# bhansconnect/alphazero-pybind11

Measured on AMD Instinct MI355X. Metric: self-play games/sec (whole node), Connect4 @ 800 MCTS sims, higher is better.
Workload: dtype bf16

## Files before the change

alphazero-pybind11_amd/csrc/dev_cache.h:

```cpp
#pragma once
#include <hip/hip_runtime.h>
#include <stdint.h>

#include <type_traits>

#include "dev_rng.h"

namespace azmi {

struct CacheView {
  uint32_t shards, cap, ghost_cap;
  uint32_t tcap, gcap;
  uint32_t np, nv;
  uint64_t* hashes;
  uint32_t* freq;
  float* policy;
  float* value;
  uint32_t* s_ring;
  uint32_t* m_ring;
  uint64_t* ghost_ring;
  uint32_t* state;
  uint64_t* map_key;
  uint32_t* map_val;
  uint64_t* gset_key;
// ... 280 lines not shown
    }
    g = uni(g);
    if (__ballot(have == cache_key(hash)) != 0ull) {
      if (g && lane == 0) __hip_atomic_store(locks + sh, 0u, __ATOMIC_RELAXED, __HIP_MEMORY_SCOPE_AGENT);
      return true;
    }
    if (g) { got = 1; break; }
    __builtin_amdgcn_s_sleep(8);
  }
  if (!got) return false;
  {
    WaveShardT<true> ws(c, sh, lane);
    const int slot = ws.insert(hash);
    if (slot >= 0) {
      const size_t e = static_cast<size_t>(sh) * kWaveCap + slot;
      if constexpr (PROBE_SAFE) {
        if (lane == 0) c_st<true>(c.hashes + e, 0ull);
        asm volatile("s_waitcnt vmcnt(0)" ::: "memory");
      }
      if (lane < c.np) c_st<true>(reinterpret_cast<uint32_t*>(c.policy) + e * c.np + lane, __float_as_uint(p_lane));
      if (lane < c.nv) c_st<true>(reinterpret_cast<uint32_t*>(c.value) + e * c.nv + lane, __float_as_uint(v_lane));
      if constexpr (PROBE_SAFE) asm volatile("s_waitcnt vmcnt(0)" ::: "memory");
      ws.store();
    }
  }
  asm volatile("s_waitcnt vmcnt(0)" ::: "memory");
  if (lane == 0) __hip_atomic_store(locks + sh, 0u, __ATOMIC_RELAXED, __HIP_MEMORY_SCOPE_AGENT);
  return true;
}

struct NoPreload { __device__ __forceinline__ void operator()() const {} };
template <int G, class F = NoPreload>
__device__ __forceinline__ int wave_shard_find(const CacheView& c, uint64_t hash, uint32_t glane, uint32_t* shard_out, F&& before_loads = F()) {
  const uint64_t k = cache_key(hash);
  const uint32_t sh = static_cast<uint32_t>(hash % c.shards);
  *shard_out = sh;
  const uint64_t* hs = c.hashes + static_cast<size_t>(sh) * kWaveCap;
  uint64_t hv[kWaveCap / G];
#pragma unroll
  for (int i = 0; i < static_cast<int>(kWaveCap) / G; ++i) hv[i] = hs[i * G + static_cast<int>(glane)];
  before_loads();
  int found = -1;
#pragma unroll
  for (int i = 0; i < static_cast<int>(kWaveCap) / G; ++i)
    if (hv[i] == k) found = i * G + static_cast<int>(glane);
  if constexpr (G == 8) {
    found = max(found, __builtin_amdgcn_update_dpp(0, found, 0xB1, 0xF, 0xF, true));
    found = max(found, __builtin_amdgcn_update_dpp(0, found, 0x4E, 0xF, 0xF, true));
    found = max(found, __builtin_amdgcn_update_dpp(0, found, 0x141, 0xF, 0xF, true));
  } else {
#pragma unroll
    for (int off = 1; off < G; off <<= 1) found = max(found, __shfl_xor(found, off, G));
  }
  return found;
}
__device__ inline void wave_shard_find_account(const CacheView& c, uint64_t hash, uint32_t sh, int slot) {
  unsigned long long* st = c.stats + static_cast<size_t>(sh) * 4;
  if (slot < 0) {
    atomicAdd(&st[1], 1ULL);
    if (c.ghost_cap > 0) {
      const uint64_t k = cache_key(hash);
      bool in_ghost = false;
      for (uint32_t i = 0; i < c.ghost_cap; ++i)
        in_ghost = in_ghost || (c.map_val[static_cast<size_t>(sh) * kWaveCap + i] &&
                                c.ghost_ring[static_cast<size_t>(sh) * c.ghost_cap + i] == k);
      if (in_ghost) atomicAdd(&st[3], 1ULL);
    }
    return;
  }
  atomicAdd(&st[0], 1ULL);
  uint32_t* f = c.freq + static_cast<size_t>(sh) * kWaveCap + slot;
  if (atomicAdd(f, 1u) >= 3u) atomicSub(f, 1u);
}


constexpr uint32_t kApplyMax = 8192;
template <uint32_t U = 8>
__device__ __forceinline__ void wave_copy_row(float* __restrict__ dst, const float* __restrict__ src, uint32_t n, uint32_t lane) {
  for (uint32_t e0 = 0; e0 < n; e0 += 64 * U) {
    float t[U];
#pragma unroll
    for (uint32_t u = 0; u < U; ++u) { const uint32_t e = e0 + u * 64 + lane; t[u] = e < n ? src[e] : 0.0f; }
#pragma unroll
    for (uint32_t u = 0; u < U; ++u) { const uint32_t e = e0 + u * 64 + lane; if (e < n) dst[e] = t[u]; }
  }
}
__device__ __forceinline__ void cache_apply_batch(const CacheView& c, const uint64_t* keys, const float* policy,
                                                   const float* value, uint32_t n, uint32_t* s_sid,
                                                   const uint8_t* groups = nullptr, uint32_t group = 0) {
  const uint32_t tid = threadIdx.x, wave = tid >> 6, lane = tid & 63;
  const uint32_t i = blockIdx.x * (blockDim.x >> 6) + wave;
  const bool own_rows = c.np <= 64 && c.nv <= 64;
  const uint64_t own_key = i < n ? keys[i] : 0ull;
  const float own_p = (i < n && own_rows && lane < c.np) ? policy[static_cast<size_t>(i) * c.np + lane] : 0.0f;
  const float own_v = (i < n && own_rows && lane < c.nv) ? value[static_cast<size_t>(i) * c.nv + lane] : 0.0f;
  for (uint32_t j = tid; j < n; j += blockDim.x) {
    const uint64_t k = (groups && groups[j] != group) ? 0 : keys[j];
    s_sid[j] = k ? static_cast<uint32_t>(k % c.shards) : 0xFFFFFFFFu;
  }
  __syncthreads();
  if (i >= n) return;
  const uint32_t my = s_sid[i];
  if (my == 0xFFFFFFFFu) return;
  bool earlier = false;
  for (uint32_t j = lane; j < i; j += 64) earlier = earlier || (s_sid[j] == my);
  if (__ballot(earlier)) return;
// ... 27 lines not shown
```

alphazero-pybind11_amd/csrc/engine_kernels.h:

```cpp
#pragma once
#include <hip/hip_runtime.h>
#include <stdint.h>

#include "dev_games.h"
#include "dev_rng.h"
#include "engine_types.h"

namespace azmi {

constexpr float kNoiseAlphaRatio = 10.83f;

__device__ __forceinline__ uint32_t seat_param(const uint32_t (&a)[4], uint32_t seat) {
  return seat == 0 ? a[0] : seat == 1 ? a[1] : seat == 2 ? a[2] : a[3];
}

__device__ __forceinline__ uint32_t gum_plan(uint32_t m, uint32_t n, uint32_t want, uint32_t& num_c_out, uint32_t& v_per_out) {
  num_c_out = 0; v_per_out = 0;
  if (m <= 1) { if (want == 0) { num_c_out = 1; v_per_out = n; } return 1; }
  uint32_t log2m = 0;
  for (uint32_t v = m - 1; v > 0; v >>= 1) ++log2m;
  if (log2m == 0) log2m = 1;
  const uint32_t d0 = n / (log2m * m);
  const uint32_t base_v = d0 > 1u ? d0 : 1u;
  uint32_t sims_used = 0, num_c = m, count = 0;
// ... 324 lines not shown
      const float sc = bcast(score_l, ci);
      if (sc > best_score) { best_score = sc; best = ci; }
    }
    return bcast(mv_l, best);
  }

  __device__ __forceinline__ bool expand_node(uint32_t seat, uint32_t node, const typename GM::State& st, uint64_t meta_keep,
                              uint32_t& c0_out, uint32_t& k_out, uint32_t* mv_out = nullptr) {
    const size_t tb = tree_base(seat);
    const uint32_t k = GM::num_valid(st);
    static_assert(GM::MAXK <= 8, "eight 4-bit move fields");
    uint32_t packed = 0;
    {
      uint32_t vm = GM::valid_mask(st), pos = 0;
      while (vm) { const uint32_t m = __builtin_ctz(vm); vm &= vm - 1; packed |= m << (4 * pos); ++pos; }
    }
    auto swap_fields = [&](uint32_t a, uint32_t b) {
      const uint32_t fa = (packed >> (4 * a)) & 0xFu, fb = (packed >> (4 * b)) & 0xFu;
      packed = (packed & ~((0xFu << (4 * a)) | (0xFu << (4 * b)))) | (fb << (4 * a)) | (fa << (4 * b));
    };
    if (k > 1) {
      uint32_t i = 1;
      if ((k & 1u) == 0) {
        const uint32_t j = lemire_below(rng, 2);
        swap_fields(i, j);
        ++i;
      }
      while (i != k) {
        const uint32_t swap_range = i + 1, b1 = swap_range + 1;
        const uint32_t x = lemire_below(rng, swap_range * b1);
        const uint32_t p0 = x / b1, p1 = x % b1;
        swap_fields(i, p0);
        ++i;
        swap_fields(i, p1);
        ++i;
      }
    }
    const uint32_t mv = lane < k ? (packed >> (4 * lane)) & 0xFu : 0u;
    const uint32_t c0 = AZMI_SEL(t_bump, seat);
    if (c0 + k > ep.cap) { raise(1u); return false; }
    if (lane < k) {
      const size_t ci = tb + c0 + lane;
      ar.nodes[ci].n = 0; ar.nodes[ci].q = 0.0f; ar.nodes[ci].pr = 0.0f; ar.nodes[ci].d = 0.0f; ar.nodes[ci].v = 0.0f;
      ar.nodes[ci].meta = meta_pack(0, 0, mv, 0, 0);
    }
#pragma unroll
    for (int p = 0; p < P; ++p) if (static_cast<uint32_t>(p) == seat) t_bump[p] = c0 + k;
    if (lane == 0)
      ar.nodes[tb + node].meta = meta_pack(c0, k, meta_mv(meta_keep), meta_player(meta_keep), meta_term(meta_keep));
    c0_out = c0;
    k_out = k;
    if (mv_out) *mv_out = mv;
    return true;
  }

  __device__ __forceinline__ uint32_t select_child(uint32_t k, uint32_t n_l, float q_l, float p_l, float v_parent,
                                   uint32_t n_parent, float fpu_reduction, uint32_t if_l = 0) const {
    return select_among(k, n_l, q_l, p_l, v_parent, select_parent(n_parent), ep.cpuct, fpu_reduction, if_l);
  }
  __device__ __forceinline__ static float select_parent(uint32_t n_parent) { return sqrtf(static_cast<float>(n_parent)); }
  __device__ __forceinline__ uint32_t select_among(uint32_t k, uint32_t n_l, float q_l, float p_l, float v_parent,
                                   float sqrt_n, float cpuct, float fpu_reduction, uint32_t if_l = 0) const {
    const float seen = seqsum8((lane < k && n_l > 0) ? p_l : 0.0f);
    const float fpu_value = v_parent - fpu_reduction * sqrtf(seen);
    float u = (n_l == 0 ? fpu_value : q_l) + cpuct * p_l * sqrt_n / static_cast<float>(n_l + if_l + 1);
    u = (u != u) ? ((lane == 0) ? __builtin_inff() : -__builtin_inff()) : u;
    u = (lane >= k) ? -__builtin_inff() : u;
    uint32_t idx = lane < k ? lane : 0xFFFFu;
    {
      float ou = dpp_f<0xB1>(u); uint32_t oi = dpp_u<0xB1>(idx);
      bool take = (ou > u) | ((ou == u) & (oi < idx));
      u = take ? ou : u; idx = take ? oi : idx;
      ou = dpp_f<0x4E>(u); oi = dpp_u<0x4E>(idx);
      take = (ou > u) | ((ou == u) & (oi < idx));
      u = take ? ou : u; idx = take ? oi : idx;
      ou = dpp_f<0x141>(u); oi = dpp_u<0x141>(idx);
      take = (ou > u) | ((ou == u) & (oi < idx));
      u = take ? ou : u; idx = take ? oi : idx;
    }
    return idx;
  }

  __device__ __forceinline__ bool find_leaf_wu(uint32_t seat, typename GM::State& leaf, uint32_t& term, uint32_t* nif) {
    sync_lanes();
    const size_t tb = tree_base(seat);
    const uint32_t root = AZMI_SEL(t_root, seat);
    cur = root; plen = 0;
    leaf = gs;
    uint64_t meta = ar.nodes[tb + cur].meta;
    uint32_t n = ar.nodes[tb + cur].n, nf = nif[cur];
    uint32_t* path = ar.path + static_cast<size_t>(slot) * ep.max_depth;
    while ((n > 0 || nf > 0) && meta_nch(meta) != 0 && meta_term(meta) == 0) {
      if (plen >= ep.max_depth) { raise(8u); return false; }
      if (lane == 0) path[plen] = cur;
      ++plen;
      const uint32_t k = meta_nch(meta), c0 = meta_ch0(meta);
      const size_t ci = tb + c0 + lane;
      uint32_t n_l = 0, if_l = 0; float q_l = 0.0f, p_l = 0.0f; uint64_t m_l = 0;
      if (lane < k) { n_l = ar.nodes[ci].n; q_l = ar.nodes[ci].q; p_l = ar.nodes[ci].pr; m_l = ar.nodes[ci].meta; if_l = nif[c0 + lane]; }
      const float fpu = (cur == root && seat_fpu_zero(seat)) ? 0.0f : ep.fpu_reduction;
      const uint32_t best = select_child(k, n_l, q_l, p_l, ar.nodes[tb + cur].v, n + nf, fpu, if_l);
      if (lane == 0) nif[cur] = nf + 1;
      cur = c0 + best;
      n = bcast(n_l, best);
      nf = bcast(if_l, best);
      meta = bcast(m_l, best);
// ... 618 lines not shown
#pragma unroll
      for (int j = 0; j < 3; ++j) { atomicAdd(reinterpret_cast<unsigned long long*>(&ar.a_cnt[j * S + slot]), static_cast<unsigned long long>(gc[j])); ar.g_cnt[j * S + slot] = 0; }
      atomicAdd(&ar.slot_games[slot], 1u);
      const uint32_t pos = atomicAdd(&ar.ctl->ended_count, 1u);
      ar.ended_list[pos] = slot;
    }
  }

  __device__ __forceinline__ void emit_leaf(const typename GM::State& leaf, uint64_t key) const {
    float* row = ar.canon + static_cast<size_t>(slot) * GM::CANON;
    for (uint32_t e = lane; e < static_cast<uint32_t>(GM::CANON); e += G) row[e] = GM::canonical_at(leaf, e);
    if (lane == 0) {
      ar.leaf_key[slot] = key;
      if (ar.leaf_pos) {
        ar.leaf_pos[0 * static_cast<size_t>(ep.S) + slot] = leaf.bb[0];
        ar.leaf_pos[1 * static_cast<size_t>(ep.S) + slot] = leaf.bb[1];
        ar.leaf_pos[2 * static_cast<size_t>(ep.S) + slot] = leaf.player;
      }
    }
  }
  struct NoEarly { __device__ __forceinline__ bool operator()(int, float&, float&) const { return false; } };
  struct NoAfter { __device__ __forceinline__ void operator()(float, float) const {} };
  template <class F = NoPreload, class E = NoEarly, class A = NoAfter>
  __device__ __forceinline__ bool cache_lookup(uint64_t key, uint32_t group, float& hit_pi, float& hit_v, F&& before_loads = F(), E&& early = E(),
                                               A&& after_hit = A()) const {
    uint32_t sh;
    const CacheView cache = ep.num_groups == 1 ? ar.cache : ar.caches[group];
    const int cslot = wave_shard_find<G>(cache, key, lane, &sh, before_loads);
    if (lane == 0) {
      unsigned long long* st = cache.stats + static_cast<size_t>(sh) * 4;
      if (cslot < 0) {
        atomicAdd(&st[1], 1ULL);
      } else {
        atomicAdd(&st[0], 1ULL);
        uint32_t* f = cache.freq + static_cast<size_t>(sh) * kWaveCap + cslot;
        atomicAdd(f, 1u);
        atomicMin(f, 3u);
      }
    }
    static_assert(M <= G, "one lane per policy entry");
    bool have = early(cslot, hit_pi, hit_v);
    if (!have) {
      if (cslot < 0) return false;
      const float* sp = cache.policy + (static_cast<size_t>(sh) * cache.cap + cslot) * M;
      const float* sv = cache.value + (static_cast<size_t>(sh) * cache.cap + cslot) * (P + 1);
      hit_pi = lane < static_cast<uint32_t>(M) ? sp[lane] : 0.0f;
      hit_v = lane <= static_cast<uint32_t>(P) ? sv[lane] : 0.0f;
      after_hit(hit_pi, hit_v);
    }
    if (lane < static_cast<uint32_t>(M)) ar.pi[static_cast<size_t>(slot) * M + lane] = hit_pi;
    if (lane <= static_cast<uint32_t>(P)) ar.v[static_cast<size_t>(slot) * (P + 1) + lane] = hit_v;
    return true;
  }
};

template <class GM, bool kPlayout = false, bool kMover = false>
__device__ __forceinline__ uint32_t round_slot(const EngineParams& ep, const EngineArrays& ar, const uint32_t slot, const uint32_t lane) {
  constexpr int G = GM::GROUP;
  constexpr int P = GM::P;
  if (slot >= ep.S) return 0xFFu;
  if (ar.ctl->stop) return 0xFFu;
  const uint8_t st = ar.sstate[slot];
  if (st == kSlotDone || st == kSlotEnded) { if (ep.cache_on && lane == 0) ar.cache_keys[slot] = 0; return 0xFFu; }
  if constexpr (!kMover) {
    if (st == kSlotQueued) {
      if (lane == 0) {
        const uint32_t group = ar.leaf_group[slot];
        if (ep.cache_on) ar.cache_keys[slot] = cache_key(ar.leaf_key[slot]);
        ar.eval_list[static_cast<size_t>(group) * ep.S + atomicAdd(&ar.ctl->eval_count[group], 1u)] = slot;
        ar.sstate[slot] = kSlotWaitEval;
      }
      return kSlotWaitEval;
    }
  }
  SlotCtx<GM> c(ep, ar, slot, lane);
  c.trace(100);
  c.load();
  if constexpr (kMover) c.flags &= ~kFlagListed;
  c.trace(101);
  uint32_t inline_sims = 0, insert_key_set = 0;
  PathRegs prec;
  bool need_process = (st == kSlotWaitEval);
  if (!need_process) {
    c.start_game();
    c.draw_capped();
    c.set_gumbel_target();
    if (ep.gumbel_on && st == kSlotRestart && !ep.tree_reuse) c.set_gumbel_num_sims(c.gs.player, 0);
  }
  bool have_regs = false;
  float reg_pi = 0.0f, reg_v = 0.0f;
  for (;;) {
    if (need_process) {
      const uint32_t cp = c.gs.player;
      const bool noise = c.seat_eps(cp) > 0 && !(c.flags & kFlagCapped);
      c.process_result(cp, (c.flags & kFlagLeafNeedsNet) != 0, noise, have_regs, reg_pi, reg_v);
      have_regs = false;
      c.trace(102);
      const uint32_t goal = (c.flags & kFlagCapped) ? c.seat_cap_visits(cp) : c.seat_visits(cp);
      if (AZMI_SEL(c.t_depth, cp) >= goal) {
        if (c.make_move(cp)) { if (ep.cache_on && lane == 0) ar.cache_keys[slot] = 0; c.store(kSlotEnded); c.trace(107); return kSlotEnded; }
        c.trace(103);
      }
    }
    const uint32_t cp = c.gs.player;
    typename GM::State leaf;
    uint32_t term = 0;
// ... 308 lines not shown
```

alphazero-pybind11_amd/csrc/pipe_types.h:

```cpp
#pragma once
#include <stdint.h>

namespace azmi {

constexpr uint32_t kReqGranules = 4;
constexpr uint32_t kResStride = 16;
constexpr uint32_t kResV = 7;
constexpr uint32_t kPipeRing = 32768;
enum PipeErr : uint32_t { kPipeErrTimeout = 1, kPipeErrRing = 2, kPipeErrTag = 4, kPipeErrLog = 8, kPipeErrLock = 16, kPipeErrSlots = 32, kPipeErrNetTimeout = 64 };

__host__ __device__ inline uint64_t pipe_lap_tag(uint32_t pos) { return static_cast<uint64_t>(((pos / kPipeRing) & 0x7FFFu) + 1u); }
__host__ __device__ inline uint64_t pipe_mix64(uint64_t x) { x ^= x >> 30; x *= 0xBF58476D1CE4E5B9ULL; x ^= x >> 27; x *= 0x94D049BB133111EBULL; x ^= x >> 31; return x; }
constexpr unsigned long long kPipeGroupSalt = 0xA5A5A5A55A5A5A5AULL;
__host__ __device__ inline uint32_t pipe_l0_entry(uint64_t key, uint32_t mask) { return static_cast<uint32_t>(pipe_mix64(key ^ 0x5851F42D4C957F2DULL)) & mask; }
__host__ __device__ inline uint32_t pipe_l0_tag(uint64_t key, uint32_t k) { return static_cast<uint32_t>(pipe_mix64(key + 0x9E3779B97F4A7C15ULL * (k + 1u)) >> 32) | 1u; }
__host__ __device__ inline uint64_t pipe_lap_tag_r(uint32_t pos, uint32_t shift) { return static_cast<uint64_t>(((pos >> shift) & 0x7FFFu) + 1u); }
constexpr unsigned long long kTokMove = 0x8000ull;
constexpr unsigned long long kTokSlotMask = 0x7FFFull;

struct PipeWg {
  uint32_t rhead;
  uint32_t rtail;
  uint32_t pad[30];
};
static_assert(sizeof(PipeWg) == 128, "one line");

struct PipeCtl {
  uint32_t head; uint32_t pad0[31];
  uint32_t tail; uint32_t pad1[31];
  uint32_t head1; uint32_t pad4[31];
  uint32_t tail1; uint32_t pad5[31];
  uint32_t err;
  uint32_t pad6[31];
  unsigned long long freezes, freeze_max;
  unsigned long long tile_hist[6];
  uint32_t pad7[16];
  uint32_t pad2a, pad2;
  unsigned long long tiles;
  unsigned long long tile_boards;
  unsigned long long epochs;
  unsigned long long sims_total;
  unsigned long long l0_hits;
  uint32_t lost_total, pad3;
  uint32_t dbg[18];
  unsigned long long prof[16];
};
static_assert(sizeof(PipeCtl) == 1024, "eight lines");

struct PipeEpoch {
  unsigned long long sims; uint32_t pad0[30];
  unsigned long long t0;
  uint32_t stop;
  uint32_t tree_done;
  uint32_t tree_arrived, net_arrived;
  uint32_t tree_late, net_late;
  uint32_t tree_late_n, net_late_n;
  uint32_t reserved[2];
  uint32_t pad1[20];
  uint32_t ins_count;
  uint32_t ended;
  uint32_t dead;
  uint32_t ins_done;
  uint32_t moved;
  uint32_t lost;
  uint32_t pad2[26];
};
static_assert(sizeof(PipeEpoch) == 384, "memset block: three lines");

struct PipeArrays {
  PipeCtl* ctl;
  PipeEpoch* ep;
  unsigned long long* ring;
  unsigned long long* ring1;
  uint32_t n_groups;
  uint32_t net_groups;
  uint32_t lock_base1;
  uint8_t* ins_grp;
  unsigned long long* rring;
  PipeWg* wg;
  uint32_t rshift;
  uint32_t big_at;
  uint32_t census_hold;
  uint32_t take_wait;
  uint32_t max_inline;
  uint32_t min_active;
  unsigned long long* res;
  unsigned long long* l0;
  uint32_t l0_mask;
  uint32_t test_drop;
// ... 16 lines not shown
```

alphazero-pybind11_amd/csrc/pipeline.hip:

```cpp
#include <hip/hip_runtime.h>

#include <chrono>
#include <mutex>
#include <cstdio>
#include <cstdlib>
#include <cstring>
#include <map>
#include <memory>

#include "../../include/azmi.h"
#include "engine_host.h"
#include "engine_kernels.h"
#include "leafnet_c4.h"
#include "pipe_types.h"

using namespace azmi;

namespace azmi {

__device__ __forceinline__ unsigned long long g_ld(const unsigned long long* p) { return __hip_atomic_load(p, __ATOMIC_RELAXED, __HIP_MEMORY_SCOPE_AGENT); }
__device__ __forceinline__ uint32_t g_ld(const uint32_t* p) { return __hip_atomic_load(p, __ATOMIC_RELAXED, __HIP_MEMORY_SCOPE_AGENT); }
__device__ __forceinline__ void g_st(unsigned long long* p, unsigned long long v) { __hip_atomic_store(p, v, __ATOMIC_RELAXED, __HIP_MEMORY_SCOPE_AGENT); }
__device__ __forceinline__ void g_st(uint32_t* p, uint32_t v) { __hip_atomic_store(p, v, __ATOMIC_RELAXED, __HIP_MEMORY_SCOPE_AGENT); }

// ... 94 lines not shown
  {
    const unsigned long long em = __ballot(on && lane == 0 && res_state == kSlotEnded);
    const unsigned long long dm = __ballot(on && lane == 0 && (res_state == kSlotDone || res_state == 0xFFu));
    const unsigned long long om = __ballot(on && lane == 0);
    const unsigned long long sm = __ballot(on && lane == 0 && was_sim != 0u);
    if (wlane == 0) {
      if (em) atomicAdd(&pe->ended, static_cast<uint32_t>(__popcll(em)));
      if (dm) atomicAdd(&pe->dead, static_cast<uint32_t>(__popcll(dm)));
      if (sm) atomicAdd(&pe->sims, static_cast<unsigned long long>(__popcll(sm)));
      atomicAdd(&pe->moved, static_cast<uint32_t>(__popcll(om)));
    }
  }
  return res_state;
}

#ifndef AZMI_TREE_MINB
#define AZMI_TREE_MINB 2
#endif
template <class GM, int NT, bool PROF, bool TWO = false, bool GUM = false>
__global__ __launch_bounds__(NT, AZMI_TREE_MINB) void k_pipe_tree(PipeKernArgs ka) {
  constexpr int G = GM::GROUP;
  constexpr int P = GM::P;
  static_assert(P == 2 && G == 8 && GM::M == 7, "written for Connect4's 8-lane groups");
  const EngineParams& ep = ka.ep;
  const EngineArrays& ar = ka.ar;
  const PipeArrays& pa = ka.pa;
  const uint32_t wlane = threadIdx.x & 63u, grp = wlane >> 3, lane0 = wlane & 7u;
  uint64_t t_start = wall_clock64(), t_last = t_start;
  PipeCtl* const pc = pa.ctl;
  PipeEpoch* const pe = pa.ep;
  PipeWg* const wc = pa.wg + blockIdx.x;
  const uint32_t rmask = (1u << pa.rshift) - 1u;
  unsigned long long* const myring = pa.rring + (static_cast<size_t>(blockIdx.x) << pa.rshift);
  if (threadIdx.x == 0) {
    unsigned long long t0 = atomicCAS(&pe->t0, 0ull, static_cast<unsigned long long>(t_start));
    if (t0 == 0ull) t0 = t_start;
    atomicMax(&pe->tree_late, static_cast<uint32_t>(t_start > t0 ? t_start - t0 : 0ull));
    const uint32_t before = atomicAdd(&pe->tree_arrived, 1u);
    asm volatile("s_waitcnt vmcnt(0)" :: "v"(before) : "memory");
  }
  __syncthreads();
  if (pa.census_hold != 0u) {
    const unsigned long long t0 = g_ld(&pe->t0);
    if (threadIdx.x == 0 && t_start > t0 && t_start - t0 >= pa.census_hold) atomicAdd(&pe->tree_late_n, 1u);
    while (wall_clock64() < t0 + pa.census_hold) __builtin_amdgcn_s_sleep(32);
    return;
  }
  bool go = g_ld(&ar.ctl->stop) == 0 && g_ld(&pc->err) == 0 && g_ld(&pe->stop) == 0;
  __shared__ uint32_t s_head;
  if (threadIdx.x == 0) s_head = wc->rhead;
  __syncthreads();
  uint64_t pf_pass = 0, pf_idle = 0, pf_n = 0, pf_act = 0, pf_polls = 0, pf_io = 0, pf_lvls = 0, pf_mv = 0;
  uint64_t pf_ph[5] = {0, 0, 0, 0, 0};
  SlotCtx<GM> c(ep, ar, 0u, lane0);

  while (go) {
    const uint64_t pf_t0 = PROF ? wall_clock64() : 0;
    uint32_t lane = lane0;
    asm volatile("" : "+v"(lane));
    c.lane = lane;
    uint32_t my_slot = kNoSlot, tok_seq = 0, tok_move = 0, n_tok = 0, empty_polls = 0, ctl_word = 0;
    uint64_t t_seen = 0;
    bool fresh_pass = true;
    for (;;) {
      const uint32_t h = __builtin_amdgcn_readfirstlane(*const_cast<volatile uint32_t*>(&s_head));
      unsigned long long tok = 0;
      bool here = false;
      if (lane == 0) {
        const uint32_t pos = h + grp;
        tok = g_ld(myring + (pos & rmask));
        here = (tok >> 48) == pipe_lap_tag_r(pos, pa.rshift);
      }
      if ((empty_polls & 3u) == 0u) {
        ctl_word = 0;
        if (wlane == 7) ctl_word = g_ld(&pe->stop) | g_ld(&pc->err) | g_ld(&ar.ctl->stop);
        else if (wlane == 15) ctl_word = g_ld(&pe->sims) >= pa.quota ? 1u : 0u;
        else if (wlane == 23) ctl_word = g_ld(&pe->ended);
        else if (wlane == 31) ctl_word = g_ld(&pe->dead);
      }
      uint32_t stop_seen = __builtin_amdgcn_readlane(ctl_word, 7) | __builtin_amdgcn_readlane(ctl_word, 15);
      {
        const uint32_t w = __builtin_amdgcn_readlane(ctl_word, 23), d = __builtin_amdgcn_readlane(ctl_word, 31);
        const uint32_t with_game = ep.S > d ? ep.S - d : 0u;
        const uint32_t thr = max(1u, static_cast<uint32_t>((static_cast<unsigned long long>(with_game) * pa.idle_num) >> 10));
        if (w >= thr || w + d >= ep.S) stop_seen = 1u;
      }
      const uint64_t now = wall_clock64();
      if (fresh_pass) { t_last = now; fresh_pass = false; }
      else pipe_freeze_credit(pc, now, t_last, t_start, wlane == 0);
      if (now - t_start > pa.soft_ticks) stop_seen = 1u;
      if (now - t_start > pa.cap_ticks) {
        if (wlane == 0) { atomicOr(&pc->err, static_cast<uint32_t>(kPipeErrTimeout)); pc->dbg[16] = __builtin_amdgcn_readlane(ctl_word, 23); pc->dbg[17] = __builtin_amdgcn_readlane(ctl_word, 31); }
        stop_seen = 1u;
      }
      if (stop_seen) {
        if (wlane == 0) g_st(&pe->stop, 1u);
        go = false;
        break;
      }
      if constexpr (PROF) pf_polls += 1;
      const unsigned long long hm = __ballot(here);
      uint32_t k = 0;
      while (k < kTreeWindow && ((hm >> (8 * k)) & 1ull)) ++k;
      if (k == 0u) { ++empty_polls; __builtin_amdgcn_s_sleep(16); continue; }
      if (k < kTreeWindow && pa.take_wait != 0u) {
        if (t_seen == 0) t_seen = now;
// ... 226 lines not shown
          uint32_t k = meta_nch(meta); const uint32_t c0 = meta_ch0(meta);
          if (k == 0) { failed = true; break; }
          const uint32_t t_node = c.bcast(fw_node, static_cast<int>(plen & 7u));
          const bool in_regs = cur == fl_node;
          const NodeRec* const cr = ar.nodes + tb + c0 + (lane < k ? lane : k - 1u);
          uint32_t n_l = cr->n; float q_l = cr->q, p_l = cr->pr, d_l = cr->d, v_l = cr->v; uint64_t m_l = cr->meta;
          float sqrt_n = SlotCtx<GM>::select_parent(n);
          asm volatile("" : "+v"(sqrt_n), "+v"(k));
          {
            const bool have = lane < k, mem = have && !in_regs;
            n_l = mem ? n_l : 0u; q_l = mem ? q_l : 0.0f; d_l = mem ? d_l : 0.0f; v_l = mem ? v_l : 0.0f;
            p_l = mem ? p_l : have ? fl_pr : 0.0f;
            m_l = mem ? m_l : have ? meta_pack(0, 0, fl_mv, 0, 0) : 0ull;
          }
          if (!in_regs) {
            if (fw && prefix && plen < fw_plen && plen < 8u) {
              const uint32_t t_n = c.bcast(fw_n, static_cast<int>(plen));
              const float t_q = c.bcast(fw_q, static_cast<int>(plen)), t_d = c.bcast(fw_d, static_cast<int>(plen)), t_v = c.bcast(fw_v, static_cast<int>(plen));
              if (c0 + lane == t_node) { n_l = t_n; q_l = t_q; d_l = t_d; v_l = t_v; if (t_node == fl_node) m_l = fl_meta; }
            }
          }
          const float fpu = (cur == root) ? fpu_root : fpu_red;
          uint32_t best;
          if constexpr (GUM) {
            if (gum_active != 0u && cur == root) best = c.gumbel_next_root_child(cp, k, n_l, q_l, p_l);
            else if (gum_active != 0u && gum_full != 0u) best = c.gumbel_interior_select(cp, k, n_l, q_l, p_l, v_cur);
            else best = c.select_among(k, n_l, q_l, p_l, v_cur, sqrt_n, cpuct, fpu);
          } else {
            best = c.select_among(k, n_l, q_l, p_l, v_cur, sqrt_n, cpuct, fpu);
          }
          const uint32_t nxt = c0 + best;
          const uint32_t s_n = c.bcast(n_l, static_cast<int>(best));
          const float s_q = c.bcast(q_l, static_cast<int>(best)), s_d = c.bcast(d_l, static_cast<int>(best)), s_v = c.bcast(v_l, static_cast<int>(best));
          const uint64_t s_m = c.bcast(m_l, static_cast<int>(best));
          if (plen < 8u) {
            if (lane == plen) { lv_node = nxt; lv_n = s_n; lv_q = s_q; lv_d = s_d; lv_v = s_v; lv_pp = meta_player(meta); }
            prefix = prefix && plen < fw_plen && nxt == t_node;
          } else {
            prefix = false;
          }
          cur = nxt; n = s_n; meta = s_m; v_cur = s_v;
          GM::play(leaf, meta_mv(meta));
          ++plen;
        }
        if (failed) { c.raise(8u); final_state = kSlotDone; st = kGrpIdle; break; }
        const uint64_t ph2 = PROF ? wall_clock64() : 0;
        if constexpr (PROF) pf_lvls += plen;
        c.cur = cur; c.plen = plen;
        rec_ok = plen <= 8u;
#pragma unroll
        for (int p = 0; p < P; ++p) if (static_cast<uint32_t>(p) == cp) c.t_tld[p] += plen;
        uint32_t term = meta_term(meta);
        lf_k = meta_nch(meta); lf_c0 = meta_ch0(meta); lf_mv = 0; lf_meta = meta;
        if (n == 0) {
          term = GM::terminal(leaf);
          const uint64_t keep = meta_pack(0, 0, meta_mv(meta), leaf.player, term);
          if (!c.expand_node(cp, cur, leaf, keep, lf_c0, lf_k, &lf_mv)) { final_state = kSlotDone; st = kGrpIdle; break; }
          lf_meta = meta_pack(lf_c0, lf_k, meta_mv(meta), leaf.player, term);
        }
        lf_term = term; lf_player = leaf.player;
        const uint64_t ph3 = PROF ? wall_clock64() : 0;
        const bool needs_net = term == 0 && !c.seat_eval_random(cp);
        c.flags = needs_net ? (c.flags | kFlagLeafNeedsNet) : (c.flags & ~kFlagLeafNeedsNet);
        if (needs_net) {
          const uint64_t key = GM::key(leaf);
          unsigned long long l0a = 0, l0b = 0;
          const uint64_t lkey = TWO ? key ^ (mg ? kPipeGroupSalt : 0ull) : key;
          const unsigned long long* const le = pa.l0 + static_cast<size_t>(pipe_l0_entry(lkey, pa.l0_mask)) * kResStride;
          const bool hit = ep.cache_on && c.cache_lookup(key, mg, reg_pi, reg_v,
            [&]() {
              if (pa.l0) {
                if (lane < static_cast<uint32_t>(GM::M)) l0a = g_ld(le + lane);
                if (lane <= static_cast<uint32_t>(P)) l0b = g_ld(le + kResV + lane);
              }
            },
            [&](int cslot, float& o_pi, float& o_v) -> bool {
              if (!pa.l0) return false;
              const bool okl = (lane >= static_cast<uint32_t>(GM::M) || static_cast<uint32_t>(l0a >> 32) == pipe_l0_tag(lkey, lane)) &&
                               (lane > static_cast<uint32_t>(P) || static_cast<uint32_t>(l0b >> 32) == pipe_l0_tag(lkey, kResV + lane));
              if (!c.group_all(okl)) return false;
              o_pi = lane < static_cast<uint32_t>(GM::M) ? __uint_as_float(static_cast<uint32_t>(l0a)) : 0.0f;
              o_v = lane <= static_cast<uint32_t>(P) ? __uint_as_float(static_cast<uint32_t>(l0b)) : 0.0f;
              if (cslot < 0) l0_hits += 1;
              return true;
            },
            [&](float h_pi, float h_v) {
              if (pa.l0 && pa.l0_wb) {
                unsigned long long* const we = pa.l0 + static_cast<size_t>(pipe_l0_entry(lkey, pa.l0_mask)) * kResStride;
                if (lane < static_cast<uint32_t>(GM::M)) g_st(we + lane, (static_cast<unsigned long long>(pipe_l0_tag(lkey, lane)) << 32) | __float_as_uint(h_pi));
                if (lane <= static_cast<uint32_t>(P)) g_st(we + kResV + lane, (static_cast<unsigned long long>(pipe_l0_tag(lkey, kResV + lane)) << 32) | __float_as_uint(h_v));
              }
            });
          if (!hit) {
            cur_key = key;
            seq = seq + 1u == 0u ? 1u : seq + 1u;
            uint32_t pos = 0;
            if (lane == 0) pos = atomicAdd(TWO ? pipe_tail_of(pc, mg) : &pc->tail, 1u);
            pos = c.template bcast_lane<0>(pos);
            const uint64_t payload = lane == 0 ? leaf.bb[0] : lane == 1 ? leaf.bb[1] : lane == 2 ? (static_cast<uint64_t>(slot) | (static_cast<uint64_t>(leaf.player) << 16))
                                                                                                  : static_cast<uint64_t>(seq);
            const unsigned long long rtag = (pa.test_drop != 0u && pos == pa.test_drop) ? pipe_lap_tag(pos + kPipeRing) : pipe_lap_tag(pos);
            if (lane < kReqGranules)
              g_st((TWO ? pipe_ring_of(pa, mg) : pa.ring) + static_cast<size_t>(pos & (kPipeRing - 1u)) * kReqGranules + lane, (rtag << 48) | (payload & kMask48));
            if (lane < 3u) ar.leaf_pos[static_cast<size_t>(lane) * ep.S + slot] = lane == 2u ? static_cast<uint64_t>(leaf.player) : payload;
            if constexpr (TWO) { if (lane == 3u) ar.leaf_group[slot] = static_cast<uint8_t>(mg); }
            st = kGrpPush;
          }
        }
        if constexpr (PROF) {
          const uint64_t ph4 = wall_clock64();
          pf_ph[0] += ph1 - ph0; pf_ph[1] += ph2 - ph1; pf_ph[2] += ph3 - ph2; pf_ph[3] += ph4 - ph3; pf_ph[4] += 1;
        }
        if (st == kGrpPush) break;
        if (++inline_sims >= pa.max_inline) break;
        if (static_cast<uint32_t>(__popcll(__ballot(lane == 0))) < pa.min_active) break;
      }
    }
    const uint64_t pf_t3 = PROF ? wall_clock64() : 0;
    if constexpr (PROF) pf_pass += pf_t3 - pf_t2;


    if (on) {
      if (st == kGrpPush) c.flags |= kFlagReqOut;
      if (lane == 0) {
        if (sims_done) ar.c_sims[slot] += sims_done;
        if (st == kGrpPush) { ar.c_evals[slot] += 1; ar.leaf_key[slot] = cur_key; }
      }
      if (rec_ok) {
        PathRegs r;
        r.node = lv_node; r.n = lv_n; r.q = lv_q; r.d = lv_d; r.v = lv_v; r.pp = lv_pp; r.mv = lf_mv; r.leaf_meta = lf_meta;
        c.store_pend(r);
        c.flags |= kFlagPendRec;
      } else {
        c.flags &= ~kFlagPendRec;
      }
      c.store(final_state);
    }
    {
      const bool tok_out = on && lane == 0 && (st == kGrpReady || listed);
      const unsigned long long rm = __ballot(tok_out);
      uint32_t base = 0;
      if (rm && wlane == 0) base = atomicAdd(&wc->rtail, static_cast<uint32_t>(__popcll(rm)));
      asm volatile("s_waitcnt vmcnt(0)" ::: "memory");
      if (on && lane == 0) g_st(ar.req_seq + slot, seq);
      if (rm) {
        base = __builtin_amdgcn_readfirstlane(base);
        if (tok_out) {
          const uint32_t pos = base + static_cast<uint32_t>(__popcll(rm & ((1ull << (grp * 8)) - 1ull)));
          g_st(myring + (pos & rmask), (pipe_lap_tag_r(pos, pa.rshift) << 48) | static_cast<unsigned long long>(slot) | (listed ? kTokMove : 0ull));
        }
      }
    }
    {
      uint32_t x = lane == 0 ? sims_done + sims_mem : 0u;
#pragma unroll
      for (int off = 32; off > 0; off >>= 1) x += __shfl_xor(x, off, 64);
      if (wlane == 0 && x) atomicAdd(&pe->sims, static_cast<unsigned long long>(x));
      if (pa.l0) {
        uint32_t y = lane == 0 ? l0_hits : 0u;
#pragma unroll
        for (int off = 32; off > 0; off >>= 1) y += __shfl_xor(y, off, 64);
        if (wlane == 0 && y) atomicAdd(&pc->l0_hits, static_cast<unsigned long long>(y));
      }
      const unsigned long long fm = __ballot(on && lane == 0 && final_state == kSlotDone);
      if (wlane == 0 && fm) atomicAdd(&pe->dead, static_cast<uint32_t>(__popcll(fm)));
    }
    if constexpr (PROF) pf_io += wall_clock64() - pf_t3;
  }

  if (wlane == 0) g_st(&pe->stop, 1u);
  if (PROF && wlane == 0) {
    atomicAdd(&pc->prof[0], pf_pass); atomicAdd(&pc->prof[1], pf_idle); atomicAdd(&pc->prof[2], pf_n); atomicAdd(&pc->prof[3], pf_act);
    atomicAdd(&pc->prof[4], pf_polls); atomicAdd(&pc->prof[5], pf_io);
    atomicAdd(&pc->prof[9], pf_ph[0]); atomicAdd(&pc->prof[10], pf_ph[1]); atomicAdd(&pc->prof[11], pf_ph[2]); atomicAdd(&pc->prof[12], pf_ph[3]);
    atomicAdd(&pc->prof[13], pf_ph[4]); atomicAdd(&pc->prof[14], pf_lvls); atomicAdd(&pc->prof[15], pf_mv); atomicAdd(&pc->prof[6], static_cast<unsigned long long>(wall_clock64() - t_start));
  }
  asm volatile("s_waitcnt vmcnt(0)" ::: "memory");
  __syncthreads();
  if (threadIdx.x == 0) { wc->rhead = s_head; atomicAdd(&pe->tree_done, 1u); }
}

template <class GM, int NT, bool DIAG = false>
__global__ __launch_bounds__(NT, 2) void k_pipe_tree_generic(PipeKernArgs ka) {
  constexpr int P = GM::P;
  const EngineParams& ep = ka.ep;
  const EngineArrays& ar = ka.ar;
  const PipeArrays& pa = ka.pa;
  const uint32_t wlane = threadIdx.x & 63u, grp = wlane >> 3, lane = wlane & 7u;
  uint64_t t_start = wall_clock64(), t_last = t_start;
  PipeCtl* const pc = pa.ctl;
  PipeEpoch* const pe = pa.ep;
  PipeWg* const wc = pa.wg + blockIdx.x;
  uint32_t* const phase_word = &wc->pad[2 + (threadIdx.x >> 6)];
  const bool diag_on = DIAG && g_ld(&pc->err) == 0u;
#define AZMI_GEN_PHASE(x) do { if (DIAG && wlane == 0 && diag_on) g_st(phase_word, static_cast<uint32_t>(x) | (static_cast<uint32_t>((wall_clock64() - t_start) / 1000u) << 8)); } while (0)
  AZMI_GEN_PHASE(1);
  if (DIAG && wlane == 0 && diag_on) g_st(&wc->pad[6 + (threadIdx.x >> 6)], static_cast<uint32_t>(t_start));
  const uint32_t rmask = (1u << pa.rshift) - 1u;
  unsigned long long* const myring = pa.rring + (static_cast<size_t>(blockIdx.x) << pa.rshift);
  if (threadIdx.x == 0) {
    unsigned long long t0 = atomicCAS(&pe->t0, 0ull, static_cast<unsigned long long>(t_start));
    if (t0 == 0ull) t0 = t_start;
    atomicMax(&pe->tree_late, static_cast<uint32_t>(t_start > t0 ? t_start - t0 : 0ull));
    const uint32_t before = atomicAdd(&pe->tree_arrived, 1u);
    asm volatile("s_waitcnt vmcnt(0)" :: "v"(before) : "memory");
  }
  __syncthreads();
  AZMI_GEN_PHASE(2);
  if (pa.census_hold != 0u) {
    const unsigned long long t0 = g_ld(&pe->t0);
    if (threadIdx.x == 0 && t_start > t0 && t_start - t0 >= pa.census_hold) atomicAdd(&pe->tree_late_n, 1u);
    while (wall_clock64() < t0 + pa.census_hold) __builtin_amdgcn_s_sleep(32);
    return;
  }
  bool go = g_ld(&ar.ctl->stop) == 0 && g_ld(&pc->err) == 0 && g_ld(&pe->stop) == 0;
  __shared__ uint32_t s_head;
  if (threadIdx.x == 0) s_head = wc->rhead;
  __syncthreads();
  const PipeKernArgs* const kargs = reinterpret_cast<const PipeKernArgs*>(reinterpret_cast<uintptr_t>(__builtin_amdgcn_kernarg_segment_ptr()));
  uint64_t seg_max[3] = {0, 0, 0}, sg_prev = DIAG ? __builtin_amdgcn_s_memtime() : 0ull;
  uint64_t ph_max[5] = {0, 0, 0, 0, 0};
  uint64_t gap_rt = 0, gap_sq = 0, sq_last = DIAG ? __builtin_amdgcn_s_memtime() : 0ull;
  uint32_t gap_where = 0, did_pass = 0, gap_polls = 0, total_polls = 0;
  while (go) {
    AZMI_GEN_PHASE(3);
    uint32_t my_slot = kNoSlot, tok_seq = 0, empty_polls = 0, ctl_word = 0;
    bool fresh_pass = true;
    for (;;) {
// ... 870 lines not shown
    AZMI_HIP_TRY(hipGetLastError());
  }
  if (!tree_only) {
    AZMI_HIP_TRY(hipEventRecord(ps->tev[4 * e + 0], ps->net_stream));
    const int rc = pipe_launch_net(ps, plan.view[0], k.tile, ps->net_launch, ps->net_stream, pa);
    if (rc != AZMI_OK) return rc;
    AZMI_HIP_TRY(hipEventRecord(ps->tev[4 * e + 1], ps->net_stream));
    AZMI_HIP_TRY(hipEventRecord(ps->ev_net, ps->net_stream));
    AZMI_HIP_TRY(hipStreamWaitEvent(st, ps->ev_net, 0));
  }
  k_pipe_settle<<<settle_blocks, 256, 0, st>>>(pm->ep, pm->ar, pa);
  AZMI_HIP_TRY(hipGetLastError());
  int rc = azmi_host_launch_move_step(pm, st);
  if (rc != AZMI_OK) return rc;
  rc = azmi_host_launch_assign(pm, st, 1u);
  if (rc != AZMI_OK) return rc;
  if (pm->ep.cache_on) {
    k_pipe_cache_insert<<<256, 256, 0, st>>>(pm->ar, pa, 1u);
    AZMI_HIP_TRY(hipGetLastError());
  }
  return AZMI_OK;
}

int pipe_finish_call(azmi_pm* pm, const PipePlan& plan, const PipeKnobs& k, uint32_t epochs, uint64_t host_enqueue_us, hipStream_t st, uint64_t* out_stats) {
  PipeState* ps = pm->pipe;
  PipeArrays& pa = ps->pa;
  const bool tree_only = plan.tree_only;
  PipeCtl hc;
  PipeEpoch he;
  AZMI_HIP_TRY(hipMemcpyAsync(&hc, pa.ctl, sizeof(hc), hipMemcpyDeviceToHost, st));
  AZMI_HIP_TRY(hipMemcpyAsync(&he, pa.ep, sizeof(he), hipMemcpyDeviceToHost, st));
  AZMI_HIP_TRY(hipStreamSynchronize(st));
  if (hc.lost_total != ps->lost_seen) {
    fprintf(stderr, "azmi_run_pipeline: %u request(s) were given up by the net side and sent again (a net workgroup fell more than half a ring behind)\n", hc.lost_total - ps->lost_seen);
    ps->lost_seen = hc.lost_total;
  }
  if (!tree_only && !hc.err) pipe_balance(ps, hc, k.balance_a, k.balance_b);
  if (out_stats) {
    out_stats[0] = hc.tiles; out_stats[1] = hc.tile_boards; out_stats[2] = he.sims; out_stats[3] = he.tree_arrived;
    out_stats[4] = he.net_arrived; out_stats[5] = he.ins_count; out_stats[6] = ps->net_launch; out_stats[7] = ps->tree_wgs;
    out_stats[8] = he.tree_late / 100u; out_stats[9] = he.net_late / 100u;
    double net_us = 0.0, tree_us = 0.0;
    for (uint32_t e = 0; e < epochs; ++e) {
      float ms = 0.0f;
      if (!tree_only && hipEventElapsedTime(&ms, ps->tev[4 * e + 0], ps->tev[4 * e + 1]) == hipSuccess) net_us += 1e3 * ms;
      if (hipEventElapsedTime(&ms, ps->tev[4 * e + 2], ps->tev[4 * e + 3]) == hipSuccess) tree_us += 1e3 * ms;
    }
    out_stats[10] = static_cast<uint64_t>(net_us); out_stats[11] = static_cast<uint64_t>(tree_us); out_stats[12] = epochs; out_stats[13] = host_enqueue_us;
    out_stats[14] = static_cast<uint64_t>(ps->calib_rounds & 0xFFu) | (static_cast<uint64_t>(std::min<unsigned long long>(hc.freezes, 0xFFFFFFull)) << 8) | (static_cast<uint64_t>(hc.lost_total) << 32);
    out_stats[15] = hc.l0_hits;
    if (k.prof) {
      fprintf(stderr, "pipe prof:");
      for (int i = 0; i < 16; ++i) fprintf(stderr, " %llu", hc.prof[i]);
      fprintf(stderr, "\n");
    }
    if (k.prof || k.hist) {
      fprintf(stderr, "pipe tile hist (tiles of 1 .. 6 boards since creation):");
      for (int i = 0; i < 6; ++i) fprintf(stderr, " %llu", hc.tile_hist[i]);
      fprintf(stderr, "\n");
    }
  }
  if (!hc.err) return AZMI_OK;
  fprintf(stderr, "pipeline dbg:");
  for (int i = 0; i < 18; ++i) fprintf(stderr, " %u", hc.dbg[i]);
  fprintf(stderr, "\n");
  if (plan.kind == 2) {
    std::vector<PipeWg> hw(ps->tree_wgs);
    if (hipMemcpy(hw.data(), pa.wg, hw.size() * sizeof(PipeWg), hipMemcpyDeviceToHost) == hipSuccess) {
      fprintf(stderr, "pipeline generic tree kernel, workgroup: rhead rtail | phase@10us of its four wavefronts | their entry times, us after wavefront 0's:");
      for (uint32_t w = 0; w < ps->tree_wgs; ++w)
        fprintf(stderr, "  [%u: %u %u | %u@%u %u@%u %u@%u %u@%u | %d %d %d]", w, hw[w].rhead, hw[w].rtail, hw[w].pad[2] & 255u, hw[w].pad[2] >> 8, hw[w].pad[3] & 255u, hw[w].pad[3] >> 8,
                hw[w].pad[4] & 255u, hw[w].pad[4] >> 8, hw[w].pad[5] & 255u, hw[w].pad[5] >> 8,
                static_cast<int32_t>(hw[w].pad[7] - hw[w].pad[6]) / 100, static_cast<int32_t>(hw[w].pad[8] - hw[w].pad[6]) / 100, static_cast<int32_t>(hw[w].pad[9] - hw[w].pad[6]) / 100);
      fprintf(stderr, "\n  wavefront 0's longest interval between two looks: wall clock x10us | SQ clock >> 10 | 0 poll loop, 1 a pass | after polls | polls in all:");
      for (uint32_t w = 0; w < ps->tree_wgs; ++w) fprintf(stderr, "  [%u: %u | %u | %u | %u | %u]", w, hw[w].pad[10], hw[w].pad[11], hw[w].pad[12], hw[w].pad[13], hw[w].pad[14]);
      fprintf(stderr, "\n  longest phases of its passes (SQ clock >> 10): publication word | granules | log ticket + drain | steps + requests | tokens:");
      for (uint32_t w = 0; w < ps->tree_wgs; ++w) fprintf(stderr, "  [%u: %u | %u | %u | %u | %u]", w, hw[w].pad[18], hw[w].pad[19], hw[w].pad[20], hw[w].pad[21], hw[w].pad[22]);
      fprintf(stderr, "\n  its longest segments (SQ clock >> 10): token load | control words | between looks:");
      for (uint32_t w = 0; w < ps->tree_wgs; ++w) fprintf(stderr, "  [%u: %u | %u | %u]", w, hw[w].pad[15], hw[w].pad[16], hw[w].pad[17]);
      fprintf(stderr, "\n");
    }
  }
  AZMI_HIP_TRY(hipMemsetAsync(&pa.ctl->err, 0, sizeof(uint32_t), st));
  AZMI_HIP_TRY(hipMemsetAsync(pa.ctl->dbg, 0, sizeof(pa.ctl->dbg), st));
  AZMI_HIP_TRY(hipStreamSynchronize(st));
  return azmi_host_fail(AZMI_ERR_STATE, "pipeline error mask 0x%x (1 a spin hit the epoch's time cap, 2 a ring entry never arrived, 4 a result tag "
                        "did not match, 8 insert log full, 16 cache lock, 32 slots, 64 the net side hit the time cap); census: %u of %u tree and %u of %u net workgroups started; "
                        "last epoch: head %u tail %u sims %llu ended %u dead %u stop %u tree_done %u tiles %llu boards %llu; latest tree / net workgroup start %u / %u us; "
                        "first time-out saw: slot %u seq %u / %u; net side: stop %u tree done %u of %u tail %u window at %u after %u0 us; "
                        "wavefronts that stood still > 2 ms (not one instruction between two looks at the clock) so far: %llu, the longest for %.1f ms",
                        hc.err, he.tree_arrived, ps->tree_wgs, he.net_arrived, ps->net_launch, hc.head, hc.tail, he.sims, he.ended, he.dead, he.stop,
                        he.tree_done, hc.tiles, hc.tile_boards, he.tree_late / 100u, he.net_late / 100u,
                        hc.dbg[1], hc.dbg[2], hc.dbg[3], hc.dbg[8], hc.dbg[9], hc.dbg[10], hc.dbg[11], hc.dbg[12], hc.dbg[13],
                        static_cast<unsigned long long>(hc.freezes), static_cast<double>(hc.freeze_max) * 1e-5);
}
}

static int run_pipeline_impl(azmi_pm* pm, azmi_net* const* nets, uint32_t num_nets, uint32_t epochs, uint64_t sims_per_epoch, void* stream, uint64_t* out_stats) {
  if (!pm) return azmi_host_fail(AZMI_ERR_INVALID, "null argument");
  const PipeKnobs k = pipe_read_knobs();
  std::lock_guard<std::recursive_mutex> lock_(pm->mu);
  std::lock_guard<std::mutex> turn_(pipeline_turn_of(pm->device));
  const PipePlan plan = pipe_plan(pm, nets, num_nets);
  if (plan.kind == 0)
    return azmi_host_fail(AZMI_ERR_STATE, "azmi_run_pipeline: the pipeline drives the Connect4 engine (no PLAYOUT seats, at most two model groups, at most %u "
                          "concurrent games) with a Connect4-family matrix-core net of one precision tier behind every model group that evaluates with a net "
// ... 192 lines not shown
```

Before: 6611.

## Issue cache and L0 probe loads before node expansion to overlap latency

```diff
diff --git a/alphazero-pybind11_amd/csrc/dev_cache.h b/alphazero-pybind11_amd/csrc/dev_cache.h
--- a/alphazero-pybind11_amd/csrc/dev_cache.h
+++ b/alphazero-pybind11_amd/csrc/dev_cache.h
@@ -356,6 +356,33 @@
 #pragma unroll
     for (int off = 1; off < G; off <<= 1) found = max(found, __shfl_xor(found, off, G));
   }
+  return found;
+}
+template <int G>
+struct ShardProbe {
+  uint32_t sh;
+  uint64_t hv[kWaveCap / G];
+};
+template <int G>
+__device__ __forceinline__ ShardProbe<G> wave_shard_issue(const CacheView& c, uint64_t hash, uint32_t glane) {
+  ShardProbe<G> p;
+  p.sh = static_cast<uint32_t>(hash % c.shards);
+  const uint64_t* hs = c.hashes + static_cast<size_t>(p.sh) * kWaveCap;
+#pragma unroll
+  for (int i = 0; i < static_cast<int>(kWaveCap) / G; ++i) p.hv[i] = hs[i * G + static_cast<int>(glane)];
+  return p;
+}
+template <int G>
+__device__ __forceinline__ int wave_shard_match(const ShardProbe<G>& p, uint64_t hash, uint32_t glane) {
+  static_assert(G == 8, "the 8-lane groups' DPP reduction");
+  const uint64_t k = cache_key(hash);
+  int found = -1;
+#pragma unroll
+  for (int i = 0; i < static_cast<int>(kWaveCap) / G; ++i)
+    if (p.hv[i] == k) found = i * G + static_cast<int>(glane);
+  found = max(found, __builtin_amdgcn_update_dpp(0, found, 0xB1, 0xF, 0xF, true));
+  found = max(found, __builtin_amdgcn_update_dpp(0, found, 0x4E, 0xF, 0xF, true));
+  found = max(found, __builtin_amdgcn_update_dpp(0, found, 0x141, 0xF, 0xF, true));
   return found;
 }
 __device__ inline void wave_shard_find_account(const CacheView& c, uint64_t hash, uint32_t sh, int slot) {
diff --git a/alphazero-pybind11_amd/csrc/engine_kernels.h b/alphazero-pybind11_amd/csrc/engine_kernels.h
--- a/alphazero-pybind11_amd/csrc/engine_kernels.h
+++ b/alphazero-pybind11_amd/csrc/engine_kernels.h
@@ -400,6 +400,55 @@
     k_out = k;
     if (mv_out) *mv_out = mv;
     return true;
+  }
+
+  struct Expansion { uint32_t mv, c0, k; };
+  __device__ __forceinline__ bool expand_draw(uint32_t seat, const typename GM::State& st, Expansion& e) {
+    const uint32_t k = GM::num_valid(st);
+    static_assert(GM::MAXK <= 8, "eight 4-bit move fields");
+    uint32_t packed = 0;
+    {
+      uint32_t vm = GM::valid_mask(st), pos = 0;
+      while (vm) { const uint32_t m = __builtin_ctz(vm); vm &= vm - 1; packed |= m << (4 * pos); ++pos; }
+    }
+    auto swap_fields = [&](uint32_t a, uint32_t b) {
+      const uint32_t fa = (packed >> (4 * a)) & 0xFu, fb = (packed >> (4 * b)) & 0xFu;
+      packed = (packed & ~((0xFu << (4 * a)) | (0xFu << (4 * b)))) | (fb << (4 * a)) | (fa << (4 * b));
+    };
+    if (k > 1) {
+      uint32_t i = 1;
+      if ((k & 1u) == 0) {
+        const uint32_t j = lemire_below(rng, 2);
+        swap_fields(i, j);
+        ++i;
+      }
+      while (i != k) {
+        const uint32_t swap_range = i + 1, b1 = swap_range + 1;
+        const uint32_t x = lemire_below(rng, swap_range * b1);
+        const uint32_t p0 = x / b1, p1 = x % b1;
+        swap_fields(i, p0);
+        ++i;
+        swap_fields(i, p1);
+        ++i;
+      }
+    }
+    e.mv = lane < k ? (packed >> (4 * lane)) & 0xFu : 0u;
+    e.c0 = AZMI_SEL(t_bump, seat);
+    e.k = k;
+    if (e.c0 + k > ep.cap) { raise(1u); return false; }
+    return true;
+  }
+  __device__ __forceinline__ void expand_commit(uint32_t seat, uint32_t node, uint64_t meta_keep, const Expansion& e) {
+    const size_t tb = tree_base(seat);
+    if (lane < e.k) {
+      const size_t ci = tb + e.c0 + lane;
+      ar.nodes[ci].n = 0; ar.nodes[ci].q = 0.0f; ar.nodes[ci].pr = 0.0f; ar.nodes[ci].d = 0.0f; ar.nodes[ci].v = 0.0f;
+      ar.nodes[ci].meta = meta_pack(0, 0, e.mv, 0, 0);
+    }
+#pragma unroll
+    for (int p = 0; p < P; ++p) if (static_cast<uint32_t>(p) == seat) t_bump[p] = e.c0 + e.k;
+    if (lane == 0)
+      ar.nodes[tb + node].meta = meta_pack(e.c0, e.k, meta_mv(meta_keep), meta_player(meta_keep), meta_term(meta_keep));
   }
 
   __device__ __forceinline__ uint32_t select_child(uint32_t k, uint32_t n_l, float q_l, float p_l, float v_parent,
@@ -1124,6 +1173,45 @@
     if (lane <= static_cast<uint32_t>(P)) ar.v[static_cast<size_t>(slot) * (P + 1) + lane] = hit_v;
     return true;
   }
+  struct CacheProbe {
+    CacheView cache;
+    ShardProbe<G> keys;
+  };
+  __device__ __forceinline__ CacheProbe probe_issue(uint64_t key, uint32_t group) const {
+    CacheProbe p;
+    p.cache = ep.num_groups == 1 ? ar.cache : ar.caches[group];
+    p.keys = wave_shard_issue<G>(p.cache, key, lane);
+    return p;
+  }
+  __device__ __forceinline__ int probe_match(const CacheProbe& p, uint64_t key) const { return wave_shard_match<G>(p.keys, key, lane); }
+  template <class E = NoEarly, class A = NoAfter>
+  __device__ __forceinline__ bool probe_finish(const CacheProbe& p, const int cslot, float& hit_pi, float& hit_v, E&& early = E(), A&& after_hit = A()) const {
+    const CacheView& cache = p.cache;
+    const uint32_t sh = p.keys.sh;
+    if (lane == 0) {
+      unsigned long long* st = cache.stats + static_cast<size_t>(sh) * 4;
+      if (cslot < 0) {
+        atomicAdd(&st[1], 1ULL);
+      } else {
+        atomicAdd(&st[0], 1ULL);
+        uint32_t* f = cache.freq + static_cast<size_t>(sh) * kWaveCap + cslot;
+        atomicAdd(f, 1u);
+        atomicMin(f, 3u);
+      }
+    }
+    bool have = early(cslot, hit_pi, hit_v);
+    if (!have) {
+      if (cslot < 0) return false;
+      const float* sp = cache.policy + (static_cast<size_t>(sh) * cache.cap + cslot) * M;
+      const float* sv = cache.value + (static_cast<size_t>(sh) * cache.cap + cslot) * (P + 1);
+      hit_pi = lane < static_cast<uint32_t>(M) ? sp[lane] : 0.0f;
+      hit_v = lane <= static_cast<uint32_t>(P) ? sv[lane] : 0.0f;
+      after_hit(hit_pi, hit_v);
+    }
+    if (lane < static_cast<uint32_t>(M)) ar.pi[static_cast<size_t>(slot) * M + lane] = hit_pi;
+    if (lane <= static_cast<uint32_t>(P)) ar.v[static_cast<size_t>(slot) * (P + 1) + lane] = hit_v;
+    return true;
+  }
 };
 
 template <class GM, bool kPlayout = false, bool kMover = false>
diff --git a/alphazero-pybind11_amd/csrc/pipe_types.h b/alphazero-pybind11_amd/csrc/pipe_types.h
--- a/alphazero-pybind11_amd/csrc/pipe_types.h
+++ b/alphazero-pybind11_amd/csrc/pipe_types.h
@@ -34,7 +34,8 @@
   uint32_t pad6[31];
   unsigned long long freezes, freeze_max;
   unsigned long long tile_hist[6];
-  uint32_t pad7[16];
+  unsigned long long prof2[4];
+  uint32_t pad7[8];
   uint32_t pad2a, pad2;
   unsigned long long tiles;
   unsigned long long tile_boards;
diff --git a/alphazero-pybind11_amd/csrc/pipeline.hip b/alphazero-pybind11_amd/csrc/pipeline.hip
--- a/alphazero-pybind11_amd/csrc/pipeline.hip
+++ b/alphazero-pybind11_amd/csrc/pipeline.hip
@@ -170,6 +170,7 @@
   __syncthreads();
   uint64_t pf_pass = 0, pf_idle = 0, pf_n = 0, pf_act = 0, pf_polls = 0, pf_io = 0, pf_lvls = 0, pf_mv = 0;
   uint64_t pf_ph[5] = {0, 0, 0, 0, 0};
+  uint64_t pf_px[3] = {0, 0, 0};
   SlotCtx<GM> c(ep, ar, 0u, lane0);
 
   while (go) {
@@ -502,36 +503,53 @@
         for (int p = 0; p < P; ++p) if (static_cast<uint32_t>(p) == cp) c.t_tld[p] += plen;
         uint32_t term = meta_term(meta);
         lf_k = meta_nch(meta); lf_c0 = meta_ch0(meta); lf_mv = 0; lf_meta = meta;
+        uint64_t key = 0, lkey = 0;
+        unsigned long long l0a = 0, l0b = 0;
+        typename SlotCtx<GM>::CacheProbe probe;
+        typename SlotCtx<GM>::Expansion ex;
+        const bool probing = n == 0 && ep.cache_on && !c.seat_eval_random(cp);
+        uint64_t keep = 0;
+        uint64_t ph_a = 0, ph_b = 0, ph_c = 0, ph_tk = 0;
         if (n == 0) {
+          key = GM::key(leaf);
+          lkey = TWO ? key ^ (mg ? kPipeGroupSalt : 0ull) : key;
+          if (probing) {
+            probe = c.probe_issue(key, mg);
+            if (pa.l0) {
+              const unsigned long long* const le = pa.l0 + static_cast<size_t>(pipe_l0_entry(lkey, pa.l0_mask)) * kResStride;
+              if (lane < static_cast<uint32_t>(GM::M)) l0a = g_ld(le + lane);
+              if (lane <= static_cast<uint32_t>(P)) l0b = g_ld(le + kResV + lane);
+            }
+          }
+          if constexpr (PROF) ph_a = wall_clock64();
           term = GM::terminal(leaf);
-          const uint64_t keep = meta_pack(0, 0, meta_mv(meta), leaf.player, term);
-          if (!c.expand_node(cp, cur, leaf, keep, lf_c0, lf_k, &lf_mv)) { final_state = kSlotDone; st = kGrpIdle; break; }
+          keep = meta_pack(0, 0, meta_mv(meta), leaf.player, term);
+          if (!c.expand_draw(cp, leaf, ex)) { final_state = kSlotDone; st = kGrpIdle; break; }
+          lf_c0 = ex.c0; lf_k = ex.k; lf_mv = ex.mv;
           lf_meta = meta_pack(lf_c0, lf_k, meta_mv(meta), leaf.player, term);
+          if constexpr (PROF) ph_b = wall_clock64();
         }
         lf_term = term; lf_player = leaf.player;
-        const uint64_t ph3 = PROF ? wall_clock64() : 0;
         const bool needs_net = term == 0 && !c.seat_eval_random(cp);
         c.flags = needs_net ? (c.flags | kFlagLeafNeedsNet) : (c.flags & ~kFlagLeafNeedsNet);
+        int cslot = -1;
+        if (needs_net && ep.cache_on) {
+          cslot = c.probe_match(probe, key);
+          if constexpr (PROF) { asm volatile("" :: "v"(cslot)); }
+        }
+        if constexpr (PROF) ph_c = wall_clock64();
+        if (n == 0) c.expand_commit(cp, cur, keep, ex);
+        const uint64_t ph3 = PROF ? wall_clock64() : 0;
         if (needs_net) {
-          const uint64_t key = GM::key(leaf);
-          unsigned long long l0a = 0, l0b = 0;
-          const uint64_t lkey = TWO ? key ^ (mg ? kPipeGroupSalt : 0ull) : key;
-          const unsigned long long* const le = pa.l0 + static_cast<size_t>(pipe_l0_entry(lkey, pa.l0_mask)) * kResStride;
-          const bool hit = ep.cache_on && c.cache_lookup(key, mg, reg_pi, reg_v,
-            [&]() {
-              if (pa.l0) {
-                if (lane < static_cast<uint32_t>(GM::M)) l0a = g_ld(le + lane);
-                if (lane <= static_cast<uint32_t>(P)) l0b = g_ld(le + kResV + lane);
-              }
-            },
-            [&](int cslot, float& o_pi, float& o_v) -> bool {
+          const bool hit = ep.cache_on && c.probe_finish(probe, cslot, reg_pi, reg_v,
+            [&](int cs, float& o_pi, float& o_v) -> bool {
               if (!pa.l0) return false;
               const bool okl = (lane >= static_cast<uint32_t>(GM::M) || static_cast<uint32_t>(l0a >> 32) == pipe_l0_tag(lkey, lane)) &&
                                (lane > static_cast<uint32_t>(P) || static_cast<uint32_t>(l0b >> 32) == pipe_l0_tag(lkey, kResV + lane));
               if (!c.group_all(okl)) return false;
               o_pi = lane < static_cast<uint32_t>(GM::M) ? __uint_as_float(static_cast<uint32_t>(l0a)) : 0.0f;
               o_v = lane <= static_cast<uint32_t>(P) ? __uint_as_float(static_cast<uint32_t>(l0b)) : 0.0f;
-              if (cslot < 0) l0_hits += 1;
+              if (cs < 0) l0_hits += 1;
               return true;
             },
             [&](float h_pi, float h_v) {
@@ -546,6 +564,7 @@
             seq = seq + 1u == 0u ? 1u : seq + 1u;
             uint32_t pos = 0;
             if (lane == 0) pos = atomicAdd(TWO ? pipe_tail_of(pc, mg) : &pc->tail, 1u);
+            if constexpr (PROF) { const uint64_t tk0 = wall_clock64(); asm volatile("s_waitcnt vmcnt(0)" : "+v"(pos) :: "memory"); ph_tk = wall_clock64() - tk0; }
             pos = c.template bcast_lane<0>(pos);
             const uint64_t payload = lane == 0 ? leaf.bb[0] : lane == 1 ? leaf.bb[1] : lane == 2 ? (static_cast<uint64_t>(slot) | (static_cast<uint64_t>(leaf.player) << 16))
                                                                                                   : static_cast<uint64_t>(seq);
@@ -559,7 +578,10 @@
         }
         if constexpr (PROF) {
           const uint64_t ph4 = wall_clock64();
-          pf_ph[0] += ph1 - ph0; pf_ph[1] += ph2 - ph1; pf_ph[2] += ph3 - ph2; pf_ph[3] += ph4 - ph3; pf_ph[4] += 1;
+          pf_ph[0] += ph1 - ph0; pf_ph[1] += ph2 - ph1; pf_ph[4] += 1;
+          if (n == 0) { pf_px[0] += ph_a - ph2; pf_ph[2] += (ph_b - ph_a) + (ph3 - ph_c); pf_px[1] += ph_c - ph_b; }
+          else pf_ph[2] += ph3 - ph2;
+          pf_ph[3] += ph4 - ph3 - ph_tk; pf_px[2] += ph_tk;
         }
         if (st == kGrpPush) break;
         if (++inline_sims >= pa.max_inline) break;
@@ -624,6 +646,7 @@
     atomicAdd(&pc->prof[4], pf_polls); atomicAdd(&pc->prof[5], pf_io);
     atomicAdd(&pc->prof[9], pf_ph[0]); atomicAdd(&pc->prof[10], pf_ph[1]); atomicAdd(&pc->prof[11], pf_ph[2]); atomicAdd(&pc->prof[12], pf_ph[3]);
     atomicAdd(&pc->prof[13], pf_ph[4]); atomicAdd(&pc->prof[14], pf_lvls); atomicAdd(&pc->prof[15], pf_mv); atomicAdd(&pc->prof[6], static_cast<unsigned long long>(wall_clock64() - t_start));
+    atomicAdd(&pc->prof2[0], pf_px[0]); atomicAdd(&pc->prof2[1], pf_px[1]); atomicAdd(&pc->prof2[2], pf_px[2]);
   }
   asm volatile("s_waitcnt vmcnt(0)" ::: "memory");
   __syncthreads();
@@ -1600,6 +1623,8 @@
     if (k.prof) {
       fprintf(stderr, "pipe prof:");
       for (int i = 0; i < 16; ++i) fprintf(stderr, " %llu", hc.prof[i]);
+      fprintf(stderr, "\npipe prof, probe (ticks issuing it, waiting for its keys, waiting for the request's ticket):");
+      for (int i = 0; i < 3; ++i) fprintf(stderr, " %llu", hc.prof2[i]);
       fprintf(stderr, "\n");
     }
     if (k.prof || k.hist) {
```

Result: slower. 6433 (-2.7%).
